# johnnovak/nim-raytracer

Measured on AMD Instinct MI355X. Metric: Mray/s (primary+shadow) on bunny.geom 1080p/256spp; 1/2/4/8-GPU scaling, higher is better.
Workload: dtype f32; 1 GPU; C3: bunny.geom baked x30 + ground plane, mesh-bunny.nim lights/camera, 1920x1080, akGrid 16x16 = 256 spp, fp32, one whole-frame call per step on one GPU; every step builds its camera-dependent data on the device; width=1920, height=1080, spp=256, triangles=69451, bvh_nodes=21204, primary_rays_per_frame=530841600, parallelism=bands1, bvh_builder=host binned SAH

## Files before the change

include/rtmi.h:

```cpp
#ifndef RTMI_H
#define RTMI_H

#include <stddef.h>
#include <stdint.h>

#ifdef __cplusplus
extern "C" {
#endif

#define RTMI_ABI_VERSION 1

enum {
  RT_OK = 0,
  RT_E_INVALID = -1,
  RT_E_UNSUPPORTED = -2,
  RT_E_DEVICE = -3,
  RT_E_NOMEM = -4,
  RT_E_IO = -5
};


enum rt_geom_type { RT_SPHERE = 0, RT_PLANE = 1, RT_BOX = 2, RT_MESH = 3 };

enum rt_light_type { RT_DISTANT_LIGHT = 0, RT_POINT_LIGHT = 1 };
// ... 63 lines not shown
  int32_t max_ray_depth;
  int32_t precision;
  uint64_t seed;
  uint32_t flags;
  uint32_t reserved;
} rt_options;

#define RT_FLAG_ANYHIT_SHADOWS 0x1u
#define RT_FLAG_COUNT_TRAVERSAL 0x2u
#define RT_FLAG_NO_REORDER 0x4u
#define RT_FLAG_NO_BINNING 0x8u
#define RT_FLAG_NO_SPLIT 0x10u
#define RT_FLAG_NO_BATCH 0x20u
#define RT_FLAG_BATCH_FALLBACK 0x40u
#define RT_FLAG_NO_LEAN1 0x80u
#define RT_FLAG_NO_GEN1 0x100u
#define RT_FLAG_NO_STATS 0x200u
#define RT_FLAG_NO_MIX 0x400u
#define RT_FLAG_TIMING 0x800u
#define RT_FLAG_NO_OBJ_BATCH 0x1000u
#define RT_FLAG_COMPACT 0x2000u
#define RT_FLAG_F64_PER_LANE 0x4000u
#define RT_FLAG_NO_UNIFORM 0x8000u

typedef struct rt_stats {
  uint64_t num_primary_rays;
  uint64_t num_intersection_tests;
  uint64_t num_intersection_hits;
  uint64_t num_shadow_rays;
  uint64_t num_reflection_rays;
} rt_stats;

typedef struct rt_traversal_counters {
  uint64_t wave_node_fetches;
  uint64_t wave_tri_fetches;
  uint64_t lane_node_visits;
  uint64_t lane_tri_tests;
} rt_traversal_counters;

typedef struct rt_scene_info {
  int64_t num_objects, num_lights, num_meshes;
  int64_t num_triangles;
  int64_t num_bvh_nodes;
  int32_t max_bvh_depth;
  int32_t device;
  int64_t device_bytes;
// ... 84 lines not shown
int rt_queue_try_recv(rt_queue *q, rt_response *out);
int rt_queue_pending(rt_queue *q);
int rt_queue_reset(rt_queue *q);
int rt_queue_shutdown(rt_queue *q);
int rt_queue_destroy(rt_queue *q);


int rt_ppm_encode_device(const float *d_fb, int32_t width, int32_t height,
                         int32_t bits, int32_t srgb, void *d_out,
                         void *hip_stream);
int64_t rt_ppm_payload_bytes(int32_t width, int32_t height, int32_t bits);
int rt_ppm_header(int32_t width, int32_t height, int32_t bits, char *buf,
                  int32_t buf_len);

int rt_rgba_encode_device(const float *d_fb, int32_t width, int32_t height,
                          uint8_t alpha, void *d_out, void *stream);

int rt_scene_last_counters(rt_scene *scene, rt_traversal_counters *out);

int rt_scene_last_split(rt_scene *scene, int64_t *lean_groups, int64_t *general_groups);
int rt_scene_last_batch(rt_scene *scene, int64_t *batched_groups, int64_t *fallback_groups);
int rt_scene_last_lean_kernel(rt_scene *scene, int32_t *kind);
int rt_scene_last_uniform(rt_scene *scene, int32_t *lit, int32_t *sky);


int rt_mat4_inverse(const double m[16], double out[16]);

int rt_load_geom(const char *path, int64_t *num_triangles, double *vertices);

#define RT_OBJ_SLASH_INDICES 0x1u
int rt_load_obj(const char *path, uint32_t flags, int64_t *num_vertices,
                double *vertices, int64_t *num_faces, int32_t *faces);

int rt_write_geom(const char *path, const double *vertices,
                  int64_t num_vertices, const int32_t *faces,
                  int64_t num_faces);

#ifdef __cplusplus
}
#endif

#endif
```

nim-raytracer_amd/csrc/rt_common.h:

```cpp
#pragma once
#include <stdint.h>
#include <stdlib.h>

namespace rtmi {

inline const char* diag_env(const char* name) {
#ifdef RTMI_DIAG
  return getenv(name);
#else
  (void)name;
  return nullptr;
#endif
}

enum : int32_t { GEOM_SPHERE = 0, GEOM_PLANE = 1, GEOM_BOX = 2, GEOM_MESH = 3 };
enum : int32_t { LIGHT_DISTANT = 0, LIGHT_POINT = 1 };
enum : int32_t { XF_IDENTITY = 0, XF_TRANSLATE = 1, XF_GENERAL = 2 };
enum : int32_t { RT_DEV_FLAG_COUNT = 0x2, RT_DEV_FLAG_FALLBACK = 0x40, RT_DEV_FLAG_NO_OBJ_BATCH = 0x1000 };

constexpr int kMaxBvhDepth = 60;
constexpr int kLeafMax = 4;
constexpr int kMaxShadeLevels = 8;
constexpr int kStatSlots = 10;

// ... 162 lines not shown
  float e2[3];
  float v0;
  float inv_h;
  float rmax;
  int32_t gu, gv;
  int32_t off_base;
  int32_t ent_base;
  int32_t pad[2];
};
static_assert(sizeof(LightGrid) == 64, "LightGrid must be 64 bytes");

struct alignas(16) FLight {
  int32_t type;
  float ci[3];
  float v[3];
  float pad;
};

constexpr uint32_t kPixCount = 0x00FFFFFFu;

constexpr int kLeanClsShift = 29;
constexpr int32_t kLeanIdxMask = (1 << kLeanClsShift) - 1;
enum : int { kUniMixed = 0, kUniLit = 1, kUniSky = 2 };

struct LTri;
struct FastParams {
  const FObj* objs;
  const FObjX* objx;
  const FMesh* meshes;
  const FLight* lights;
  const BvhNode* tree;
  const float* normals;
  const int32_t* pix_slots;
  const uint32_t* pix_cnt;
  const LightGrid* grids;
  const int32_t* grid_off;
  const int32_t* grid_ent;
  const unsigned long long* obj_pix;
  const LightGrid* obj_grids;
  const unsigned long long* obj_grid_mask;
  unsigned long long obj_off_grid;
  const uint32_t* pix_info;
  float* fb;
  unsigned long long* partials;
  unsigned int* queue;
  const int32_t* order;
// ... 96 lines not shown
```

nim-raytracer_amd/csrc/rt_fast.h:

```cpp
#pragma once
#include <hip/hip_runtime.h>

#include "rt_common.h"
#include "rt_sampling.h"

#ifndef RT_CONST
#if defined(__HIP_DEVICE_COMPILE__)
#define RT_CONST __attribute__((address_space(4)))
#else
#define RT_CONST
#endif
#endif



#include "rt_occupancy.h"

namespace rtmi {
namespace fast {

enum : unsigned {
  F_SPHERE = 1u, F_BOX = 2u, F_PLANE = 4u, F_MESH = 8u,
  F_XF_GENERAL = 16u,
  F_POINT = 32u,
// ... 2069 lines not shown
        irr_add(E[k], L.ci, vis ? fmaxf(dot3(N[k], sd), 0.0f) : 0.0f);
      }
    }
  }
  p = params();
  const RT_CONST FObjX& mx = at(p->objx, mesh);
  const RT_CONST FObjX& px_ = at(p->objx, po);
  const F3 am = f3(mx.albedo_pi[0], mx.albedo_pi[1], mx.albedo_pi[2]);
  const F3 ap = f3(px_.albedo_pi[0], px_.albedo_pi[1], px_.albedo_pi[2]);
  const F3 bg = f3(p->bg[0], p->bg[1], p->bg[2]);
#pragma unroll
  for (int k = 0; k < S; ++k) {
    const bool lt = lane_in(litm[k]);
    const F3 alb = f3(hm[k] ? am.x : ap.x, hm[k] ? am.y : ap.y, hm[k] ? am.z : ap.z);
    const F3 a = mul3(alb, E[k]);
    acc_add3(acc, lt ? a.x : bg.x, lt ? a.y : bg.y, lt ? a.z : bg.z);
  }
  wi.v[STAT_PRIMARY] += (unsigned)(64 * S);
  wi.v[STAT_SHADOW] += (unsigned)NL * nlit;
  wi.v[STAT_HITS] += wave_sum(hitl);
  return true;
}

template <unsigned F>
__device__ __forceinline__ LdsF* sample_table(KP p, const GroupPix& gp, float* sample_lds, int wib, int L) {
  LdsF* tb = nullptr;
  if ((F & F_STOCHASTIC) && p->aa_kind >= 3) {
    const int m = p->grid_m, spp = p->spp;
    const uint64_t key = rng_pixel_key(p->seed, gp.x, gp.y);
    tb = (LdsF*)sample_lds + ((size_t)(wib * (64 / L) + (lane_id_fresh() >> p->log2_lanes)) * 2 * spp);
    volatile LdsF* t = tb;
    for (int e = gp.sub; e < spp; e += L) {
      double a, b;
      canonical_entry(key, m, e, a, b);
      t[e] = (float)a;
      t[spp + e] = (float)b;
    }
    const uint64_t bx = 2 * (uint64_t)spp;
    const uint64_t by = bx + (p->aa_kind == 3 ? (uint64_t)spp : (uint64_t)m);
    if (gp.sub < m) {
      const int i = gp.sub;
      for (int j = 0; j < m; ++j) {
        const int k = rng_pick(rng_draw(key, p->aa_kind == 3 ? bx + (uint64_t)j * m + i : bx + (uint64_t)j), j, m);
        const float a = t[j * m + i], b = t[k * m + i];
        t[j * m + i] = b;
        t[k * m + i] = a;
// ... 930 lines not shown
    }
    qj = __builtin_amdgcn_readfirstlane(qj_next);
    if (lane == 0) qj_next = (int)atomicAdd(head, 1u);
    g = qj * p->shards + shard;
  }
  p = params();
  const int lane = (int)__lane_id();
  flush_stats(ws, lds_tot[wib], lane);
  const int wave = (int)(blockIdx.x * (blockDim.x >> 6) + threadIdx.x / 64u);
  if (lane < kStatSlots) p->partials[(size_t)wave * kStatSlots + lane] = lds_tot[wib][lane];
}

#ifndef RTMI_GEN1_WAVES
#define RTMI_GEN1_WAVES 7
#endif
template <int NL>
__device__ __forceinline__ void gen1_loop(KP p, LdsF* ls, Stats32& ws, unsigned long long* tot, int& nflush) {
  constexpr unsigned F = F_PLANE | F_MESH;
  WorkQ<RTMI_GEN_RUN> wq;
  int g = wq.start(p->queue, p->shards, list_items(p->list_n, p->ngroups, 1));
  while (g >= 0) {
    p = params();
    const int iters = p->iters;
    const int gg = cp(p->order)[g];
    GroupPix gp = group_pixel(p, gg, lane_id_fresh());
    gp.valid = true;
    gp.x = __builtin_amdgcn_readfirstlane(gp.x);
    gp.y = __builtin_amdgcn_readfirstlane(gp.y);
    gp.out_row = __builtin_amdgcn_readfirstlane(gp.out_row);
    const int pu = __builtin_amdgcn_readfirstlane(gp.y * p->width + gp.x);
    const unsigned pinfo = at(p->pix_info, pu);
    Acc acc;
    acc.v = f3(0.0f, 0.0f, 0.0f);
    Stats32 wi;
#pragma unroll
    for (int k = 0; k < kStatSlots; ++k) wi.v[k] = 0u;
    bool ok = (pinfo & kPixCount) <= (1u << p->slot_lg);
    for (int it = 0; ok && it < iters; it += kGenBatch) ok = gen1_batch<kGenBatch, NL>(p, gp, pu, it, pinfo, acc, wi);
    if (params()->flags & RT_DEV_FLAG_FALLBACK) ok = false;
    if (ok) {
      ws.v[STAT_PRIMARY] += wi.v[STAT_PRIMARY];
      ws.v[STAT_SHADOW] += wi.v[STAT_SHADOW];
      ws.v[STAT_HITS] += wi.v[STAT_HITS];
#if defined(RTMI_DIAG_GEN_COUNT) || defined(RTMI_DIAG_LANES)
      for (int q = STAT_NODE_FETCH; q <= STAT_LANE_TRIS; ++q) ws.v[q] += wi.v[q];
#endif
    } else {
      acc.v = f3(0.0f, 0.0f, 0.0f);
      ws.v[STAT_GEN_FALLBACK] += 1u;
      for (int i2 = 0; i2 < iters; ++i2) {
        p = params();
        const int s = i2 * 64 + gp.sub;
        const F3 d = camera_dir<F>(p, gp, s, nullptr);
        const F3 o = f3(p->cam[0], p->cam[1], p->cam[2]);
        ws.v[STAT_PRIMARY] += 64u;
        shade_path<false, F, false>(p, o, d, true, gp.y * p->width + gp.x, pinfo, ls, acc, ws);
      }
    }
    p = params();
    finish_item(p, gp, acc.v, 64);
    const int lane = lane_id_fresh();
// ... 58 lines not shown
```

nim-raytracer_amd/csrc/rt_frame.h:

```cpp
#pragma once
#include <stdint.h>

#include "rt_bins_geom.h"
#include "rt_common.h"

namespace rtmi {

constexpr int kFrameMaxPlanes = 8;

struct FrameRows {
  int32_t mode, y0, nrows, step, band_h, rank, world, height;
};
__host__ __device__ inline bool frame_has_row(const FrameRows& r, int y) {
  if (y < 0 || y >= r.height) return false;
  if (r.mode == 0) {
    const int d = y - r.y0;
    return d >= 0 && d < r.nrows * r.step && d % r.step == 0;
  }
  return (y / r.band_h) % r.world == r.rank;
}
__host__ __device__ inline bool frame_meets_rows(const FrameRows& r, int ylo, int yhi) {
  ylo = ylo < 0 ? 0 : ylo;
  yhi = yhi < r.height - 1 ? yhi : r.height - 1;
  if (ylo > yhi) return false;
// ... 38 lines not shown
struct HugeFace {
  int32_t rec, pad;
  int32_t r[4];
  double pr[6];
};

struct RecordsLaunch {
  int32_t mode, y0, nrows, ncols, step, max_step, band_h, rank, world, width, height, ngroups;
  uint32_t* info;
  int32_t nplanes, nl;
  uint32_t have;
  bg::SkipCam cam;
  bg::SkipPlaneC planes[kFrameMaxPlanes];
  const LightGrid* grids;
  const int32_t* sat;
  int64_t sat_off[8];
  int32_t records;
  int32_t split;
  uint32_t full;
  int32_t* lean;
  int32_t* heavy;
  int32_t* ctr;
  bg::UniformCam uni;
  uint32_t* uni_cls;
};

struct FrameLaunch {
  const DevBinTri* tris;
  int32_t nf;
  bg::PixCam cam;
  FrameRows rows;
  int32_t* cnt;
  int32_t* slots;
  int32_t slot_lg;
  HugeFace* huge;
  int32_t parity;
  RecordsLaunch r;
  uint8_t* tile_bits;
  unsigned long long* tile_cls;
  int32_t tiles_x, ntiles;
  unsigned int* zero;
  int32_t nzero;
  int32_t diag;
};

struct DevObjBox {
// ... 24 lines not shown
```

nim-raytracer_amd/csrc/rt_frame.hip:

```cpp
#include <cstdlib>
#include <hip/hip_runtime.h>

#include <algorithm>

#include "rt_bins.h"
#include "rt_frame.h"

namespace rtmi {
namespace {

__device__ __forceinline__ unsigned lane_rank(unsigned long long m) {
  return __builtin_amdgcn_mbcnt_hi((unsigned)(m >> 32), __builtin_amdgcn_mbcnt_lo((unsigned)m, 0u));
}

struct LaunchPix {
  int x, y;
  bool valid, drawn;
};
__device__ __forceinline__ LaunchPix launch_pixel(const RecordsLaunch& a, int j, int k) {
  LaunchPix r;
  r.x = j * a.step;
  r.valid = j < a.ncols && k < a.nrows;
  if (a.mode == 0) {
    r.y = a.y0 + k * a.step;
// ... 257 lines not shown
  for (int off = 32; off >= 1; off >>= 1) {
    const unsigned lo = (unsigned)__shfl_xor((int)(unsigned)v, off);
    const unsigned hi = (unsigned)__shfl_xor((int)(unsigned)(v >> 32), off);
    v += ((unsigned long long)hi << 32) | lo;
  }
  if (lane == 0) wpart[w] = v;
  int cls[kChunkTiles];
#pragma unroll
  for (int i = 0; i < kChunkTiles; ++i) {
    cls[i] = px[i].valid ? pixel_class(r, px[i], inf[i]) : 0;
    const unsigned long long ml = __ballot(cls[i] == 1), mh = __ballot(cls[i] == 2);
    if (lane == 0) wsum[i][w] = ((unsigned long long)__popcll(ml) << 32) | __popcll(mh);
  }
  __syncthreads();
  unsigned long long base = wpart[0] + wpart[1] + wpart[2] + wpart[3];
#pragma unroll
  for (int i = 0; i < kChunkTiles; ++i) {
    const int t = t0 + i;
    const unsigned long long ml = __ballot(cls[i] == 1), mh = __ballot(cls[i] == 2);
    unsigned long long b = base;
    for (int q = 0; q < w; ++q) b += wsum[i][q];
    const int bx = t % a.tiles_x, by = t / a.tiles_x;
    const int g = (by * kTileH + w) * r.ncols + bx * kTileW + lane;
    const int uc = r.uni.on && cls[i] == 1 ? bg::uniform_class(r.uni, px[i].x, px[i].y) : kUniMixed;
    const unsigned long long mul = __ballot(uc == kUniLit), mus = __ballot(uc == kUniSky);
    if (r.uni.on && lane == 0 && t < a.ntiles)
      r.uni_cls[t * kTileH + w] = (uint32_t)__popcll(mul) << 16 | (uint32_t)__popcll(mus);
    if (cls[i] == 1) r.lean[(int)(b >> 32) + (int)lane_rank(ml)] = g | (uc << kLeanClsShift);
    if (cls[i] == 2) r.heavy[(int)(b & 0xffffffffull) + (int)lane_rank(mh)] = g;
    base += wsum[i][0] + wsum[i][1] + wsum[i][2] + wsum[i][3];
  }
  if ((int)blockIdx.x == (int)gridDim.x - 1) {
    const int nl = (int)(base >> 32), nh = (int)(base & 0xffffffffull);
    if (tid == 0) {
      r.ctr[FC_LEAN] = nl;
      r.ctr[FC_HEAVY] = nh;
    }
    const int end = nl == 0 ? 64 : (nl + 63) / 64 * 64;
    for (int e = nl + tid; e < end; e += 256) r.lean[e] = -1;
  }
}

__global__ __launch_bounds__(512) void k_frame_obj_rects(const ObjMaskLaunch a) {
  __shared__ int alw[64];
  const int t = (int)threadIdx.x, i = t >> 3, c = t & 7;
  bool proj = false, bad = false;
  double px = 0.0, py = 0.0;
  if (i < a.nobj) {
    const DevObjBox& b = a.objs[i];
    proj = !b.always;
    const double pw[3] = {(c & 1) ? b.hi[0] : b.lo[0], (c & 2) ? b.hi[1] : b.lo[1], (c & 4) ? b.hi[2] : b.lo[2]};
    double pc[3];
// ... 108 lines not shown
```

nim-raytracer_amd/csrc/rtmi.cpp:

```cpp
#include <hip/hip_runtime.h>

#include <algorithm>
#include <array>
#include <atomic>
#include <chrono>
#include <cmath>
#include <cstdarg>
#include <cstdio>
#include <cstdlib>
#include <cstring>
#include <memory>
#include <mutex>
#include <set>
#include <thread>
#include <string>
#include <vector>

#include "../../include/rtmi.h"
#include "rt_bins.h"
#include "rt_bvh.h"
#include "rt_common.h"
#include "rt_frame.h"

using namespace rtmi;
// ... 210 lines not shown
  bool has_grids = false;
  std::vector<GridOcc> grid_occ;
  std::vector<LightGridHost> grid_host;
  std::vector<SkipPlane> skip_planes;
  bool skippable = false;
  DevBuf<DevBinTri> bin_dev;
  double mesh_lo[3] = {0, 0, 0}, mesh_hi[3] = {0, 0, 0};
  DevBuf<int32_t> sat_dev;
  int64_t sat_off[8] = {};
  struct Frame {
    int w = 0, h = 0;
    DevBuf<int32_t> cnt, slots, lean, heavy, ctr, orect;
    DevBuf<uint32_t> info, uni_cls;
    int uni_rows = 0;
    DevBuf<unsigned long long> omask, status;
    DevBuf<HugeFace> huge;
    DevBuf<unsigned char> tiles;
    int slot_lg = -1;
    int want_lg = slot_lg_env();
    uint32_t calls = 0;
    bool counted = false;
    bool listed = false;
    bool uniform = false;
    hipEvent_t built = nullptr;
    hipEvent_t used = nullptr;
    bool used_rec = false;
    int id = 0;
    void invalidate() { w = h = 0; }
    size_t bytes() const {
      return cnt.bytes() + slots.bytes() + lean.bytes() + heavy.bytes() + ctr.bytes() + orect.bytes() +
             info.bytes() + uni_cls.bytes() + omask.bytes() + status.bytes() + huge.bytes() + tiles.bytes();
    }
    void release() {
      cnt.release(); slots.release(); lean.release(); heavy.release(); ctr.release(); orect.release();
      info.release(); uni_cls.release(); omask.release(); status.release(); huge.release(); tiles.release();
      slot_lg = -1;
      w = h = 0;
    }
  } fr, fr2;
  std::vector<ObjBox> obj_boxes;
  bool objbins = false;
  DevBuf<LightGrid> obj_grids;
  DevBuf<unsigned long long> obj_grid_mask;
  unsigned long long obj_off_grid = 0;
  bool has_obj_grids = false;
  DevBuf<DevObjBox> objbox_dev;
// ... 1070 lines not shown
  u.on = 1;
  u.m = p.grid_m;
  u.cam_a = p.cam_a;
  u.cam_b = p.cam_b;
  u.cam_c = p.cam_c;
  u.cam_d = p.cam_d;
  u.c4 = p.cam[4];
  u.c7 = p.cam[7];
  u.c10 = p.cam[10];
  u.st = p.sample_step;
  u.of = p.sample_off;
  u.nroy = nroy;
  bool ok = p.bias >= 1e-30f &&
            (double)p.bias > 16.0 * 1.1920928955078125e-7 *
                                 ((double)std::fabs(oy) + (double)std::fabs(ty) + (double)std::fabs(nroy));
  for (int l = 0; l < p.nlight; ++l) {
    const float sdy = -s->h_light_vy[(size_t)l];
    ok = ok && sdy > 1e-6f && sdy <= 1e6f;
  }
  u.lit_ok = ok ? 1 : 0;
}

void records_launch(rt_scene* s, const rt_options* o, const Mapping& mp, const FastParams& p, bool records,
                    bool split, bool uniform, RecordsLaunch& r) {
  std::memset(&r, 0, sizeof r);
  r.mode = mp.mode;
  r.y0 = mp.y0;
  r.nrows = mp.nrows;
  r.ncols = mp.ncols;
  r.step = mp.step;
  r.max_step = mp.max_step;
  r.band_h = mp.band_h;
  r.rank = mp.rank;
  r.world = mp.world;
  r.width = o->width;
  r.height = o->height;
  r.ngroups = p.ngroups;
  r.info = s->fr.info.p;
  r.records = records ? 1 : 0;
  if (records && s->skippable && s->skip_planes.size() <= (size_t)kFrameMaxPlanes) {
    std::vector<bg::SkipPlaneC> pcs;
    if (skip_camera(s->skip_planes, s->mesh_w2o, s->c2w, s->fov, o->width, o->height, o->bias, &r.cam, &pcs)) {
      r.nplanes = (int32_t)pcs.size();
      std::copy(pcs.begin(), pcs.end(), r.planes);
      r.nl = std::min(8, s->nlight);
      for (int l = 0; l < r.nl; ++l) r.have |= s->grid_occ[(size_t)l].g.gu > 0 ? 1u << l : 0u;
      r.grids = s->grids.p;
      r.sat = s->sat_dev.p;
      for (int l = 0; l < 8; ++l) r.sat_off[l] = s->sat_off[l];
    }
  }
  r.split = split ? 1 : 0;
  r.full = s->nlight >= 32 ? ~0u : (1u << s->nlight) - 1u;
  r.lean = s->fr.lean.p;
  r.heavy = s->fr.heavy.p;
  r.ctr = s->fr.ctr.p;
  if (split && uniform) {
    uniform_cam(s, p, r.uni);
    r.uni_cls = s->fr.uni_cls.p;
  }
}

int frame_build(rt_scene* s, const rt_options* o, const Mapping& mp, const FastParams& p, bool records, bool split,
                bool uniform, unsigned int* zero, int nzero, hipStream_t st, bool* ok, bool* zeroed) {
  *ok = false;
  *zeroed = false;
  if (!s->binnable || s->bin_tris.empty()) return RT_OK;
  FrameLaunch a;
  std::memset(&a, 0, sizeof a);
  if (!pixel_camera(s->mesh_o2w, s->mesh_w2o, s->c2w, s->fov, o->width, o->height, &a.cam)) return RT_OK;
  for (int c = 0; c < 8; ++c) {
    const double q[3] = {(c & 1) ? s->mesh_hi[0] : s->mesh_lo[0], (c & 2) ? s->mesh_hi[1] : s->mesh_lo[1],
                         (c & 4) ? s->mesh_hi[2] : s->mesh_lo[2]};
    double pw[3], pc[3];
    bg::xform_point(s->mesh_o2w, q, pw);
    bg::xform_point(a.cam.w2c, pw, pc);
    if (!(pc[2] < -1e-9 * (1.0 + std::fabs(pc[0]) + std::fabs(pc[1])))) return RT_OK;
  }
  int rc = frame_buffers(s, o->width, o->height, st);
  if (rc) return rc;
  rt_scene::Frame& f = s->fr;
  a.tris = s->bin_dev.p;
  a.nf = (int32_t)s->bin_tris.size();
  a.rows = frame_rows(mp, o->height);
  a.cnt = f.cnt.p;
  a.slots = f.slots.p;
  a.slot_lg = f.slot_lg;
  a.huge = f.huge.p;
  a.parity = (int32_t)(f.calls++ & 1u);
  records_launch(s, o, mp, p, records, split, uniform, a.r);
  a.tile_bits = f.tiles.p;
  a.tile_cls = f.status.p;
  static const int diag_b2 = rtmi::diag_env("RTMI_DIAG_B2") ? std::atoi(rtmi::diag_env("RTMI_DIAG_B2")) : 0;
  a.diag = diag_b2;
  a.tiles_x = (mp.ncols + 63) / 64;
  a.ntiles = a.tiles_x * ((mp.nrows + 3) / 4);
  a.zero = zero;
  a.nzero = nzero;
  if ((rc = rtmi_frame_build(&a, st))) {
    f.invalidate();
    return fail(RT_E_DEVICE, "frame build launch failed: %s", hipGetErrorString((hipError_t)rc));
  }
  f.listed = true;
  f.uniform = a.r.uni.on != 0;
  f.uni_rows = a.ntiles * 4;
  *zeroed = zero != nullptr;
  *ok = true;
  return RT_OK;
}

int frame_obj_masks(rt_scene* s, const rt_options* o, const Mapping& mp, hipStream_t st, bool* ok) {
  *ok = false;
  ObjMaskLaunch a;
  std::memset(&a, 0, sizeof a);
  static const double kIdentity[16] = {1, 0, 0, 0, 0, 1, 0, 0, 0, 0, 1, 0, 0, 0, 0, 1};
  bg::PixCam pc;
  if (!pixel_camera(kIdentity, kIdentity, s->c2w, s->fov, o->width, o->height, &pc)) return RT_OK;
  int rc = frame_buffers(s, o->width, o->height, st);
  if (rc) return rc;
  a.objs = s->objbox_dev.p;
  a.nobj = s->nobj;
  a.width = o->width;
  a.height = o->height;
  std::memcpy(a.w2c, pc.w2c, sizeof a.w2c);
  a.cam_a = pc.cam_a;
  a.cam_c = pc.cam_c;
  a.margin = kPixelMargin;
// ... 133 lines not shown
  if (!binning || pl.L < 16 || !sampler_in_pixel(o->aa_kind)) return RT_OK;
  int rc;
  bool lists = false, masks = false;
  static const char* cost_dump = rtmi::diag_env("RTMI_COST_DUMP");
  const unsigned sub = f32_subset(s, o);
  const bool want_split = !(o->flags & (RT_FLAG_NO_SPLIT | RT_FLAG_COUNT_TRAVERSAL)) && !p.cost && !cost_dump &&
                          s->nlight <= 8 && rtmi_lean_f32_blocks_per_cu(sub, f32_table_lds(s, o)) > 0;
  const bool records = pl.L == 64;
  *split = records && want_split && !p.order;
  hipStream_t bs = st;
  if (s->pipe) {
    bs = s->bstream;
    if (s->fr.used_rec) HIP_TRY(hipStreamWaitEvent(bs, s->fr.used, 0));
  }
  auto join = [&]() -> int {
    if (bs != st) {
      HIP_TRY(hipEventRecord(s->fr.built, bs));
      HIP_TRY(hipStreamWaitEvent(st, s->fr.built, 0));
    }
    return RT_OK;
  };
  const bool uniform = *split && lean1_ok(s, o, p, sub) && !(o->flags & (RT_FLAG_NO_LEAN1 | RT_FLAG_NO_UNIFORM)) &&
                       rtmi_lean1_quads() && (long long)mp.ncols * mp.nrows <= (long long)kLeanIdxMask;
  if ((rc = frame_build(s, o, mp, p, records, *split, uniform, zero, nzero, bs, &lists, zeroed))) {
    join();
    return rc;
  }
  if (lists) {
    p.pix_slots = s->fr.slots.p;
    p.pix_cnt = s->fr.info.p;
    p.slot_lg = s->fr.slot_lg;
    if (records) p.pix_info = s->fr.info.p;
  } else {
    *split = false;
  }
  if (s->objbins) {
    if ((rc = frame_obj_masks(s, o, mp, bs, &masks))) {
      join();
      return rc;
    }
    if (masks) p.obj_pix = s->fr.omask.p;
  }
  return join();
}

template <class R>
void fill_params(rt_scene* s, const PrecisionData<R>& pd, const rt_options* o, const Mapping& mp, float* fb,
// ... 73 lines not shown

bool mix_policy() {
  static const int force = rtmi::diag_env("RTMI_MIX") ? std::atoi(rtmi::diag_env("RTMI_MIX")) : -1;
  return force != 0;
}

bool lean1_ok(const rt_scene* s, const rt_options* o, const FastParams& p, unsigned sub) {
  return sub == SUB_MESH && p.nobj == 2 && p.shadow_mesh >= 0 &&
         (p.nlight == 1 || p.nlight == 2) && !p.has_point_light && p.aa_kind == RT_AA_GRID &&
         p.log2_grid_m >= 0 && p.log2_grid_m <= 6 && p.lanes_per_px == 64 && p.spp % 256 == 0 &&
         p.iters * 64 == p.spp && p.iters % 4 == 0 && s->nobj == 2;
}

int launch(rt_scene* s, const rt_options* o, const Mapping& mp, float* d_out, hipStream_t st, bool reduce,
           unsigned int* zero, int nzero) {
  int blocks = 1;
  auto clear = [&]() -> int {
    if (nzero > 0) HIP_TRY(hipMemsetAsync(zero, 0, (size_t)nzero * sizeof(unsigned int), st));
    return RT_OK;
  };
  s->fr.counted = false;
  s->fr.listed = false;
  s->fr.uniform = false;
  s->pending_reduce = 0;
  s->last_lean = 0;
  s->last_lean_kind = 0;
  s->last_general = 0;
  s->last_batched = 0;
  if (o->precision == RT_FP64) {
    if (int rc = clear()) return rc;
    RenderParams<double> p;
    fill_params<double>(s, s->f64, o, mp, d_out, p, &blocks);
    s->last_general = p.ngroups;
    if (p.ngroups == 0) return RT_OK;
    if (p.aa_kind >= RT_AA_JITTERED) {
      const size_t need = (size_t)blocks * 256 * 2 * (size_t)p.spp;
      if (s->f64_tables.n < need) {
        HIP_TRY(hipStreamSynchronize(st));
        int rc = s->f64_tables.alloc(need);
        if (rc) return rc;
      }
      p.sample_scratch = s->f64_tables.p;
    }
    s->last_lean = 0;
    s->last_lean_kind = 0;
    s->last_general = p.ngroups;
    s->last_batched = 0;
    const bool binning = !(o->flags & (RT_FLAG_NO_BINNING | RT_FLAG_COUNT_TRAVERSAL));
    bool lists = false;
    if (binning && sampler_in_pixel(o->aa_kind) && s->skippable) {
      FastParams pf;
      std::memset(&pf, 0, sizeof pf);
      bool zeroed = false;
      if (int rc = frame_build(s, o, mp, pf, true, false, false, nullptr, 0, st, &lists, &zeroed)) return rc;
      if (lists) p.pix_info = s->fr.info.p;
    }
    const int px64 = o->aa_kind == RT_AA_GRID && p.spp >= 64 && !(o->flags & (RT_FLAG_F64_PER_LANE | RT_FLAG_COUNT_TRAVERSAL))
                         ? (s->any_reflective && o->max_ray_depth >= 1 ? 2 : 1)
                         : 0;
    if (px64) {
      if (lists) {
        p.pix_slots = s->fr.slots.p;
        p.slot_lg = s->fr.slot_lg;
        p.lean_plane = s->lean64_plane;
      }
      if (binning && s->has_grids) {
        p.grids = s->grids.p;
        p.grid_off = s->grid_off.p;
        p.grid_ent = s->grid_ent.p;
        if (!s->sh64_ready && s->shadow_mesh >= 0) {
          if (int rc = s->sh64.alloc(s->grid_ent.n)) return rc;
          for (int li = 0; li < s->nlight && li < (int)s->grid_host.size(); ++li) {
            const LightGridHost& lg = s->grid_host[(size_t)li];
            if (lg.g.gu <= 0 || lg.ent.empty()) continue;
            const int e = rtmi_build_sh64(s->f64.objects.p, s->shadow_mesh, s->f64.lights.p, li,
                                          s->grid_ent.p + lg.g.ent_base, (int)lg.ent.size(), s->f64.tris.p,
                                          (int32_t)s->num_nodes, s->sh64.p + lg.g.ent_base, st);
// ... 412 lines not shown
  *general = c[FC_HEAVY];
  return RT_OK;
}
}

extern "C" int rt_scene_last_split(rt_scene* s, int64_t* lean_groups, int64_t* general_groups) {
  if (!s || !lean_groups || !general_groups) return fail(RT_E_INVALID, "null argument");
  std::lock_guard<std::mutex> lk(s->mu);
  return last_lists(s, lean_groups, general_groups);
}

extern "C" int rt_scene_last_uniform(rt_scene* s, int32_t* lit, int32_t* sky) {
  if (!s || !lit || !sky) return fail(RT_E_INVALID, "null argument");
  std::lock_guard<std::mutex> lk(s->mu);
  *lit = 0;
  *sky = 0;
  if (!s->fr.counted || !s->fr.uniform) return RT_OK;
  DeviceGuard g(s->device);
  std::vector<uint32_t> c((size_t)s->fr.uni_rows);
  HIP_TRY(hipEventSynchronize(s->done));
  HIP_TRY(hipMemcpy(c.data(), s->fr.uni_cls.p, c.size() * sizeof(uint32_t), hipMemcpyDeviceToHost));
  for (const uint32_t v : c) {
    *lit += (int32_t)(v >> 16);
    *sky += (int32_t)(v & 0xffffu);
  }
  return RT_OK;
}

extern "C" int rt_scene_last_lean_kernel(rt_scene* s, int32_t* kind) {
  if (!s || !kind) return fail(RT_E_INVALID, "null argument");
  std::lock_guard<std::mutex> lk(s->mu);
  *kind = s->last_lean_kind;
  return RT_OK;
}

extern "C" int rt_scene_last_batch(rt_scene* s, int64_t* batched_groups, int64_t* fallback_groups) {
  if (!s || !batched_groups || !fallback_groups) return fail(RT_E_INVALID, "null argument");
  std::lock_guard<std::mutex> lk(s->mu);
  *batched_groups = s->last_batched;
  if (s->last_batched < 0) {
    int64_t lean = 0;
    const int rc = last_lists(s, &lean, batched_groups);
    if (rc) return rc;
  }
  *fallback_groups = s->last_fallback;
  return RT_OK;
}

// ... 96 lines not shown
```

nim-raytracer_amd/rtmi/abi.py:

```python
import ctypes as C

RTMI_ABI_VERSION = 1

RT_OK = 0
RT_E_INVALID = -1
RT_E_UNSUPPORTED = -2
RT_E_DEVICE = -3
RT_E_NOMEM = -4
RT_E_IO = -5

RT_SPHERE, RT_PLANE, RT_BOX, RT_MESH = 0, 1, 2, 3
RT_DISTANT_LIGHT, RT_POINT_LIGHT = 0, 1
RT_AA_NONE, RT_AA_GRID, RT_AA_JITTERED, RT_AA_MULTI_JITTERED, RT_AA_CORRELATED_MULTI_JITTERED = range(5)
RT_FP32, RT_FP64 = 0, 1
RT_FLAG_ANYHIT_SHADOWS = 0x1
RT_FLAG_COUNT_TRAVERSAL = 0x2
RT_FLAG_NO_REORDER = 0x4
RT_FLAG_NO_BINNING = 0x8
RT_FLAG_NO_SPLIT = 0x10
RT_FLAG_NO_BATCH = 0x20
RT_FLAG_BATCH_FALLBACK = 0x40
RT_FLAG_NO_LEAN1 = 0x80
RT_FLAG_NO_GEN1 = 0x100
RT_FLAG_NO_STATS = 0x200
RT_FLAG_NO_MIX = 0x400
RT_FLAG_TIMING = 0x800
RT_FLAG_NO_OBJ_BATCH = 0x1000
RT_FLAG_COMPACT = 0x2000
RT_FLAG_F64_PER_LANE = 0x4000
RT_FLAG_NO_UNIFORM = 0x8000
RT_BVH_SAH = 0
RT_OBJ_SLASH_INDICES = 0x1
RT_BVH_PLOC = 1

_d16 = C.c_double * 16
_d3 = C.c_double * 3


class rt_mesh_desc(C.Structure):
    _fields_ = [
        ("vertices", C.POINTER(C.c_double)),
        ("num_vertices", C.c_int64),
        ("faces", C.POINTER(C.c_int32)),
        ("num_faces", C.c_int64),
        ("normals", C.POINTER(C.c_double)),
    ]


class rt_object_desc(C.Structure):
    _fields_ = [
        ("type", C.c_int32),
        ("mesh", C.c_int32),
        ("object_to_world", _d16),
# ... 106 lines not shown
    "rt_version": (C.c_int, []),
    "rt_build_source_hash": (C.c_char_p, []),
    "rt_last_error": (C.c_char_p, []),
    "rt_init": (C.c_int, [C.c_int]),
    "rt_device_count": (C.c_int, []),
    "rt_scene_create": (C.c_int, [C.POINTER(rt_scene_desc), C.POINTER(_P)]),
    "rt_scene_destroy": (C.c_int, [_P]),
    "rt_scene_get_info": (C.c_int, [_P, C.POINTER(rt_scene_info)]),
    "rt_scene_set_camera": (C.c_int, [_P, C.POINTER(C.c_double), C.c_double]),
    "rt_render_lines": (C.c_int, [_P, C.POINTER(rt_options), C.POINTER(C.c_float), C.c_int32,
                                  C.c_int32, C.c_int32, C.c_int32, C.c_int32, C.c_int32,
                                  C.POINTER(rt_stats)]),
    "rt_render_lines_device": (C.c_int, [_P, C.POINTER(rt_options), _P, C.c_int32, C.c_int32,
                                         C.c_int32, C.c_int32, _P, C.POINTER(rt_stats)]),
    "rt_render_bands_device": (C.c_int, [_P, C.POINTER(rt_options), _P, C.c_int32, C.c_int32,
                                         C.c_int32, _P, C.POINTER(rt_stats)]),
    "rt_unshard_bands_device": (C.c_int, [_P, _P, C.c_int32, C.c_int32, C.c_int32, C.c_int32, _P]),
    "rt_band_rows": (C.c_int, [C.c_int32, C.c_int32, C.c_int32, C.POINTER(C.c_int32)]),
    "rt_scene_last_counters": (C.c_int, [_P, C.POINTER(rt_traversal_counters)]),
    "rt_scene_last_split": (C.c_int, [_P, C.POINTER(C.c_int64), C.POINTER(C.c_int64)]),
    "rt_scene_last_lean_kernel": (C.c_int, [_P, C.POINTER(C.c_int32)]),
    "rt_scene_last_batch": (C.c_int, [_P, C.POINTER(C.c_int64), C.POINTER(C.c_int64)]),
    "rt_scene_last_uniform": (C.c_int, [_P, C.POINTER(C.c_int32), C.POINTER(C.c_int32)]),
    "rt_mat4_inverse": (C.c_int, [C.POINTER(C.c_double), C.POINTER(C.c_double)]),
    "rt_load_geom": (C.c_int, [C.c_char_p, C.POINTER(C.c_int64), C.POINTER(C.c_double)]),
    "rt_ppm_encode_device": (C.c_int, [_P, C.c_int32, C.c_int32, C.c_int32, C.c_int32, _P, _P]),
    "rt_ppm_payload_bytes": (C.c_int64, [C.c_int32, C.c_int32, C.c_int32]),
    "rt_rgba_encode_device": (C.c_int, [_P, C.c_int32, C.c_int32, C.c_uint8, _P, _P]),
    "rt_ppm_header": (C.c_int, [C.c_int32, C.c_int32, C.c_int32, C.c_char_p, C.c_int32]),
    "rt_load_obj": (C.c_int, [C.c_char_p, C.c_uint32, C.POINTER(C.c_int64), C.POINTER(C.c_double),
                              C.POINTER(C.c_int64), C.POINTER(C.c_int32)]),
    "rt_write_geom": (C.c_int, [C.c_char_p, C.POINTER(C.c_double), C.c_int64, C.POINTER(C.c_int32), C.c_int64]),
    "rt_scene_last_stats": (C.c_int, [_P, C.POINTER(rt_stats)]),
    "rt_scene_last_timing": (C.c_int, [_P, C.POINTER(C.c_double), C.POINTER(C.c_double)]),
    "rt_multi_create": (C.c_int, [C.POINTER(rt_scene_desc), C.POINTER(C.c_int32), C.c_int32, C.c_int32,
                                  C.POINTER(_P)]),
    "rt_render_frame_multi_device": (C.c_int, [_P, C.POINTER(rt_options), _P, C.POINTER(rt_stats)]),
    "rt_render_frame_multi": (C.c_int, [_P, C.POINTER(rt_options), C.POINTER(C.c_float), C.c_int32, C.c_int32,
                                        C.POINTER(rt_stats)]),
    "rt_multi_set_camera": (C.c_int, [_P, C.POINTER(C.c_double), C.c_double]),
    "rt_multi_destroy": (C.c_int, [_P]),
    "rt_queue_create": (C.c_int, [_P, C.POINTER(_P)]),
    "rt_queue_start": (C.c_int, [_P]),
    "rt_queue_stop": (C.c_int, [_P]),
    "rt_queue_state": (C.c_int, [_P]),
    "rt_queue_is_ready": (C.c_int, [_P]),
# ... 20 lines not shown
```

nim-raytracer_amd/rtmi/renderer.py:

```python
import contextlib
import ctypes as C
import threading

import numpy as np

from . import abi, glm
from ._lib import RtmiError, check, lib
from .scene import Options, Scene, Stats, flatten


def initRenderer(device=0):
    check(lib().rt_init(int(device)))


def device_count():
    return int(lib().rt_device_count())


class DeviceScene:

    def __init__(self, scene: Scene, device=0, bvh_builder=abi.RT_BVH_SAH):
        initRenderer(device)
        self.device = device
        self.scene = scene
# ... 56 lines not shown
        check(lib().rt_render_bands_device(self.h, C.byref(o), C.c_void_p(ptr), int(band_h), int(rank),
                                           int(world), _stream(stream), C.byref(st) if stats else None))
        return Stats.from_c(st) if stats else None

    def last_pipelined(self):
        f = lib().rtmi_test_last_pipelined
        f.restype = C.c_int
        f.argtypes = [C.c_void_p, C.POINTER(C.c_int32)]
        s = C.c_int32()
        r = f(self.h, C.byref(s))
        if r < 0:
            raise RuntimeError("rtmi_test_last_pipelined failed")
        return bool(r)

    def last_split(self):
        a, b = C.c_int64(), C.c_int64()
        check(lib().rt_scene_last_split(self.h, C.byref(a), C.byref(b)))
        return int(a.value), int(b.value)

    def last_uniform(self):
        a, b = C.c_int32(), C.c_int32()
        check(lib().rt_scene_last_uniform(self.h, C.byref(a), C.byref(b)))
        return int(a.value), int(b.value)

    def last_lean_kernel(self):
        k = C.c_int32()
        check(lib().rt_scene_last_lean_kernel(self.h, C.byref(k)))
        return int(k.value) & 15

    def last_compacted(self):
        k = C.c_int32()
        check(lib().rt_scene_last_lean_kernel(self.h, C.byref(k)))
        return bool(int(k.value) & 16)

    def last_lean_lanes(self):
        k = C.c_int32()
        check(lib().rt_scene_last_lean_kernel(self.h, C.byref(k)))
        return int(k.value) >> 8

    def last_batch(self):
        a, b = C.c_int64(), C.c_int64()
        check(lib().rt_scene_last_batch(self.h, C.byref(a), C.byref(b)))
        return int(a.value), int(b.value)

    def last_timing(self):
        a, b = C.c_double(), C.c_double()
# ... 353 lines not shown
```

Before: 2.316 million Mray/s.

## Add ground-plane fast path for general pixel groups that only see the floor

During frame list building, heavy (general) pixel groups whose footprint is classified as uniformly lit ground are tagged with a ground bit. The general kernel then sends these groups to a specialized ground1_batch routine. It computes the plane hit analytically and traces only shadow rays through the light grid, skipping full primary BVH traversal and the generic shading path. The trade-offs are extra per-group classification work, a new code path with fallbacks when the grid is unsafe, and repacked uniform-class counters (the sky count now uses 8 bits).

```diff
diff --git a/include/rtmi.h b/include/rtmi.h
--- a/include/rtmi.h
+++ b/include/rtmi.h
@@ -109,6 +109,7 @@
 #define RT_FLAG_COMPACT 0x2000u
 #define RT_FLAG_F64_PER_LANE 0x4000u
 #define RT_FLAG_NO_UNIFORM 0x8000u
+#define RT_FLAG_NO_GROUND1 0x10000u
 
 typedef struct rt_stats {
   uint64_t num_primary_rays;
@@ -239,6 +240,7 @@
 int rt_scene_last_batch(rt_scene *scene, int64_t *batched_groups, int64_t *fallback_groups);
 int rt_scene_last_lean_kernel(rt_scene *scene, int32_t *kind);
 int rt_scene_last_uniform(rt_scene *scene, int32_t *lit, int32_t *sky);
+int rt_scene_last_ground(rt_scene *scene, int32_t *ground);
 
 
 int rt_mat4_inverse(const double m[16], double out[16]);
diff --git a/nim-raytracer_amd/csrc/rt_common.h b/nim-raytracer_amd/csrc/rt_common.h
--- a/nim-raytracer_amd/csrc/rt_common.h
+++ b/nim-raytracer_amd/csrc/rt_common.h
@@ -208,6 +208,7 @@
 constexpr int kLeanClsShift = 29;
 constexpr int32_t kLeanIdxMask = (1 << kLeanClsShift) - 1;
 enum : int { kUniMixed = 0, kUniLit = 1, kUniSky = 2 };
+constexpr int32_t kGenGroundBit = 1 << kLeanClsShift;
 
 struct LTri;
 struct FastParams {
diff --git a/nim-raytracer_amd/csrc/rt_fast.h b/nim-raytracer_amd/csrc/rt_fast.h
--- a/nim-raytracer_amd/csrc/rt_fast.h
+++ b/nim-raytracer_amd/csrc/rt_fast.h
@@ -2115,6 +2115,138 @@
   return true;
 }
 
+#ifndef RTMI_GROUND_BATCH
+#define RTMI_GROUND_BATCH 4
+#endif
+constexpr int kGroundBatch = RTMI_GROUND_BATCH;
+static_assert(kGroundBatch == 1 || kGroundBatch == 2 || kGroundBatch == 4, "iters is a multiple of 4");
+template <int S, int NL>
+__device__ __forceinline__ bool ground1_batch(KP p, const GroupPix& gp, int it0, unsigned pinfo, Acc& acc,
+                                              Stats32& wi) {
+  p = params();
+  const int mesh = p->shadow_mesh, po = 1 - mesh;
+  const FObj mob = at(p->objs, mesh);
+  F3 ro[S];
+  {
+    const F3 o = f3(p->cam[0], p->cam[1], p->cam[2]);
+    const float nroy = -(o.y + at(p->objs, po).t[1]), bias = p->bias;
+    const int mm = p->grid_m - 1, lg = p->log2_grid_m;
+    const float st = p->sample_step, of = p->sample_off;
+    const float px = (float)gp.x + __builtin_fmaf((float)(gp.sub & mm), st, of);
+    const float cx = (px - p->cam_b) * p->cam_a;
+    const float q0 = __builtin_fmaf(cx, cx, 1.0f);
+    const float ax = __builtin_fmaf(cx, p->cam[3], -p->cam[9]), ay = __builtin_fmaf(cx, p->cam[4], -p->cam[10]),
+                az = __builtin_fmaf(cx, p->cam[5], -p->cam[11]);
+#pragma unroll
+    for (int k = 0; k < S; ++k) {
+      const int s = (it0 + k) * 64 + gp.sub;
+      const float py = (float)gp.y + __builtin_fmaf((float)(s >> lg), st, of);
+      const float cy = (p->cam_d - py) * p->cam_c;
+      const float rl = rsq(__builtin_fmaf(cy, cy, q0));
+      const F3 d = f3(__builtin_fmaf(cy, p->cam[6], ax) * rl, __builtin_fmaf(cy, p->cam[7], ay) * rl,
+                      __builtin_fmaf(cy, p->cam[8], az) * rl);
+      const float th = nroy * rcp(d.y);
+      const F3 hw = f3(__builtin_fmaf(d.x, th, o.x), __builtin_fmaf(d.y, th, o.y), __builtin_fmaf(d.z, th, o.z));
+      const F3 so = f3(__builtin_fmaf(0.0f, bias, hw.x), __builtin_fmaf(1.0f, bias, hw.y),
+                       __builtin_fmaf(0.0f, bias, hw.z));
+      ro[k] = f3(so.x + mob.t[0], so.y + mob.t[1], so.z + mob.t[2]);
+    }
+  }
+  unsigned long long occ[NL][S];
+  unsigned nocc = 0u;
+  const unsigned skipw = pinfo >> 24;
+#pragma unroll
+  for (int li = 0; li < NL; ++li) {
+#pragma unroll
+    for (int k = 0; k < S; ++k) occ[li][k] = 0ull;
+    if (((skipw >> li) & 1u) != 0u || mob.root < 0) continue;
+    p = params();
+    const FLight L = at(p->lights, li);
+    const F3 sd = f3(-L.v[0], -L.v[1], -L.v[2]);
+    unsigned long long pm[S], anyp = 0ull;
+#pragma unroll
+    for (int k = 0; k < S; ++k) {
+      pm[k] = bal(mesh_gate(mob, slab_ray(ro[k], sd)));
+      anyp |= pm[k];
+    }
+    if (anyp == 0ull) continue;
+    const KP q = params();
+    if (!q->grids || q->grids[li].gu <= 0) return false;
+    const RT_CONST LightGrid& G = cp(q->grids)[li];
+    F3 rd[S];
+    float stop[S], tc[S], best[S];
+    unsigned long long unused[S];
+    int cell[S];
+    unsigned long long todo[S], left = 0ull, unsafe = 0ull;
+#pragma unroll
+    for (int k = 0; k < S; ++k) {
+      const bool part = lane_in(pm[k]);
+      rd[k] = sd;
+      stop[k] = __uint_as_float(__float_as_uint(finf()) - 1u);
+      tc[k] = part ? finf() : -1.0f;
+      best[k] = part ? finf() : 0.0f;
+      unused[k] = 0ull;
+      const F3 r = ro[k];
+      const float gu = __builtin_fmaf(r.x, G.e1[0], __builtin_fmaf(r.y, G.e1[1], r.z * G.e1[2]));
+      const float gv = __builtin_fmaf(r.x, G.e2[0], __builtin_fmaf(r.y, G.e2[1], r.z * G.e2[2]));
+      const float fu = (gu - G.u0) * G.inv_h, fv = (gv - G.v0) * G.inv_h;
+      const bool safe = fmaxf(fmaxf(fabsf(r.x), fabsf(r.y)), fabsf(r.z)) <= G.rmax;
+      const bool on = fu >= 0.0f && fu < (float)G.gu && fv >= 0.0f && fv < (float)G.gv;
+      cell[k] = safe && on ? G.off_base + (int)fv * G.gu + (int)fu : -1;
+      todo[k] = bal(part && cell[k] >= 0);
+      unsafe |= bal(part && !safe);
+      left |= todo[k];
+    }
+    if (unsafe != 0ull) return false;
+    const int32_t* bent = q->grid_ent + G.ent_base;
+    while (left != 0ull) {
+      int kb = -1;
+#pragma unroll
+      for (int k = S - 1; k >= 0; --k)
+        if (todo[k]) kb = __builtin_amdgcn_readlane(cell[k], (int)__builtin_ctzll(todo[k]));
+      unsigned fl = 0u;
+      unsigned long long own[S];
+      left = 0ull;
+#pragma unroll
+      for (int k = 0; k < S; ++k) {
+        own[k] = bal(cell[k] == kb) & todo[k];
+        todo[k] &= ~own[k];
+        left |= todo[k];
+        fl |= own[k] != 0ull ? (1u << k) : 0u;
+      }
+      (void)list_search_batch<S, false>(q, bent, cp(q->grid_off)[kb], cp(q->grid_off)[kb + 1], fl, ro, rd, stop, own,
+                                        unused, best, tc, nullptr, grid_rec_of(q, li, G));
+    }
+#pragma unroll
+    for (int k = 0; k < S; ++k) {
+      occ[li][k] = pm[k] & bal(__float_as_uint(best[k]) != __float_as_uint(finf()));
+      nocc += pc(occ[li][k]);
+    }
+  }
+  p = params();
+  F3 E[S];
+#pragma unroll
+  for (int k = 0; k < S; ++k) E[k] = f3(0.0f, 0.0f, 0.0f);
+#pragma unroll
+  for (int li = 0; li < NL; ++li) {
+    const FLight L = at(p->lights, li);
+    const float ndl = fmaxf(dot3(f3(0.0f, 1.0f, 0.0f), f3(-L.v[0], -L.v[1], -L.v[2])), 0.0f);
+#pragma unroll
+    for (int k = 0; k < S; ++k) irr_add(E[k], L.ci, lane_in(occ[li][k]) ? 0.0f : ndl);
+  }
+  const RT_CONST FObjX& px_ = at(p->objx, po);
+  const F3 ap = f3(px_.albedo_pi[0], px_.albedo_pi[1], px_.albedo_pi[2]);
+#pragma unroll
+  for (int k = 0; k < S; ++k) {
+    const F3 a = mul3(ap, E[k]);
+    acc_add3(acc, a.x, a.y, a.z);
+  }
+  wi.v[STAT_PRIMARY] += (unsigned)(64 * S);
+  wi.v[STAT_SHADOW] += (unsigned)(NL * 64 * S);
+  wi.v[STAT_HITS] += (unsigned)(64 * S) + nocc;
+  return true;
+}
+
 template <unsigned F>
 __device__ __forceinline__ LdsF* sample_table(KP p, const GroupPix& gp, float* sample_lds, int wib, int L) {
   LdsF* tb = nullptr;
@@ -3091,7 +3223,15 @@
   while (g >= 0) {
     p = params();
     const int iters = p->iters;
-    const int gg = cp(p->order)[g];
+    const int ge = cp(p->order)[g];
+    const bool gnd = (ge & kGenGroundBit) != 0 && p->ngroups <= kLeanIdxMask;
+    const int gg = gnd ? ge & kLeanIdxMask : ge;
+#ifdef RTMI_DIAG_NOGROUND
+    if (gnd) {
+      g = wq.next();
+      continue;
+    }
+#endif
     GroupPix gp = group_pixel(p, gg, lane_id_fresh());
     gp.valid = true;
     gp.x = __builtin_amdgcn_readfirstlane(gp.x);
@@ -3105,7 +3245,11 @@
 #pragma unroll
     for (int k = 0; k < kStatSlots; ++k) wi.v[k] = 0u;
     bool ok = (pinfo & kPixCount) <= (1u << p->slot_lg);
-    for (int it = 0; ok && it < iters; it += kGenBatch) ok = gen1_batch<kGenBatch, NL>(p, gp, pu, it, pinfo, acc, wi);
+    if (gnd) {
+      for (int it = 0; ok && it < iters; it += kGroundBatch) ok = ground1_batch<kGroundBatch, NL>(p, gp, it, pinfo, acc, wi);
+    } else {
+      for (int it = 0; ok && it < iters; it += kGenBatch) ok = gen1_batch<kGenBatch, NL>(p, gp, pu, it, pinfo, acc, wi);
+    }
     if (params()->flags & RT_DEV_FLAG_FALLBACK) ok = false;
     if (ok) {
       ws.v[STAT_PRIMARY] += wi.v[STAT_PRIMARY];
diff --git a/nim-raytracer_amd/csrc/rt_frame.h b/nim-raytracer_amd/csrc/rt_frame.h
--- a/nim-raytracer_amd/csrc/rt_frame.h
+++ b/nim-raytracer_amd/csrc/rt_frame.h
@@ -84,6 +84,7 @@
   int32_t* heavy;
   int32_t* ctr;
   bg::UniformCam uni;
+  int32_t ground;
   uint32_t* uni_cls;
 };
 
diff --git a/nim-raytracer_amd/csrc/rt_frame.hip b/nim-raytracer_amd/csrc/rt_frame.hip
--- a/nim-raytracer_amd/csrc/rt_frame.hip
+++ b/nim-raytracer_amd/csrc/rt_frame.hip
@@ -303,12 +303,15 @@
     for (int q = 0; q < w; ++q) b += wsum[i][q];
     const int bx = t % a.tiles_x, by = t / a.tiles_x;
     const int g = (by * kTileH + w) * r.ncols + bx * kTileW + lane;
-    const int uc = r.uni.on && cls[i] == 1 ? bg::uniform_class(r.uni, px[i].x, px[i].y) : kUniMixed;
-    const unsigned long long mul = __ballot(uc == kUniLit), mus = __ballot(uc == kUniSky);
-    if (r.uni.on && lane == 0 && t < a.ntiles)
-      r.uni_cls[t * kTileH + w] = (uint32_t)__popcll(mul) << 16 | (uint32_t)__popcll(mus);
+    const bool lean_c = r.uni.on && cls[i] == 1, gen_c = r.ground && cls[i] == 2 && (inf[i] & kPixCount) == 0u;
+    const int uc = lean_c || gen_c ? bg::uniform_class(r.uni, px[i].x, px[i].y) : kUniMixed;
+    const bool gnd = gen_c && uc == kUniLit;
+    const unsigned long long mul = __ballot(lean_c && uc == kUniLit), mus = __ballot(lean_c && uc == kUniSky);
+    const unsigned long long mug = __ballot(gnd);
+    if ((r.uni.on || r.ground) && lane == 0 && t < a.ntiles)
+      r.uni_cls[t * kTileH + w] = (uint32_t)__popcll(mul) << 16 | (uint32_t)__popcll(mug) << 8 | (uint32_t)__popcll(mus);
     if (cls[i] == 1) r.lean[(int)(b >> 32) + (int)lane_rank(ml)] = g | (uc << kLeanClsShift);
-    if (cls[i] == 2) r.heavy[(int)(b & 0xffffffffull) + (int)lane_rank(mh)] = g;
+    if (cls[i] == 2) r.heavy[(int)(b & 0xffffffffull) + (int)lane_rank(mh)] = gnd ? g | kGenGroundBit : g;
     base += wsum[i][0] + wsum[i][1] + wsum[i][2] + wsum[i][3];
   }
   if ((int)blockIdx.x == (int)gridDim.x - 1) {
diff --git a/nim-raytracer_amd/csrc/rtmi.cpp b/nim-raytracer_amd/csrc/rtmi.cpp
--- a/nim-raytracer_amd/csrc/rtmi.cpp
+++ b/nim-raytracer_amd/csrc/rtmi.cpp
@@ -256,6 +256,7 @@
     bool counted = false;
     bool listed = false;
     bool uniform = false;
+    bool ground = false;
     hipEvent_t built = nullptr;
     hipEvent_t used = nullptr;
     bool used_rec = false;
@@ -1372,7 +1373,7 @@
 }
 
 void records_launch(rt_scene* s, const rt_options* o, const Mapping& mp, const FastParams& p, bool records,
-                    bool split, bool uniform, RecordsLaunch& r) {
+                    bool split, bool uniform, bool ground, RecordsLaunch& r) {
   std::memset(&r, 0, sizeof r);
   r.mode = mp.mode;
   r.y0 = mp.y0;
@@ -1405,14 +1406,16 @@
   r.lean = s->fr.lean.p;
   r.heavy = s->fr.heavy.p;
   r.ctr = s->fr.ctr.p;
-  if (split && uniform) {
+  if (split && (uniform || ground)) {
     uniform_cam(s, p, r.uni);
+    r.uni.on = uniform ? 1 : 0;
+    r.ground = ground ? 1 : 0;
     r.uni_cls = s->fr.uni_cls.p;
   }
 }
 
 int frame_build(rt_scene* s, const rt_options* o, const Mapping& mp, const FastParams& p, bool records, bool split,
-                bool uniform, unsigned int* zero, int nzero, hipStream_t st, bool* ok, bool* zeroed) {
+                bool uniform, bool ground, unsigned int* zero, int nzero, hipStream_t st, bool* ok, bool* zeroed) {
   *ok = false;
   *zeroed = false;
   if (!s->binnable || s->bin_tris.empty()) return RT_OK;
@@ -1438,7 +1441,7 @@
   a.slot_lg = f.slot_lg;
   a.huge = f.huge.p;
   a.parity = (int32_t)(f.calls++ & 1u);
-  records_launch(s, o, mp, p, records, split, uniform, a.r);
+  records_launch(s, o, mp, p, records, split, uniform, ground, a.r);
   a.tile_bits = f.tiles.p;
   a.tile_cls = f.status.p;
   static const int diag_b2 = rtmi::diag_env("RTMI_DIAG_B2") ? std::atoi(rtmi::diag_env("RTMI_DIAG_B2")) : 0;
@@ -1453,6 +1456,7 @@
   }
   f.listed = true;
   f.uniform = a.r.uni.on != 0;
+  f.ground = a.r.ground != 0;
   f.uni_rows = a.ntiles * 4;
   *zeroed = zero != nullptr;
   *ok = true;
@@ -1632,7 +1636,11 @@
   };
   const bool uniform = *split && lean1_ok(s, o, p, sub) && !(o->flags & (RT_FLAG_NO_LEAN1 | RT_FLAG_NO_UNIFORM)) &&
                        rtmi_lean1_quads() && (long long)mp.ncols * mp.nrows <= (long long)kLeanIdxMask;
-  if ((rc = frame_build(s, o, mp, p, records, *split, uniform, zero, nzero, bs, &lists, zeroed))) {
+  const bool ground = *split && lean1_ok(s, o, p, sub) &&
+                      !(o->flags & (RT_FLAG_NO_BATCH | RT_FLAG_NO_GEN1 | RT_FLAG_NO_GROUND1)) && p.grids &&
+                      rtmi_gen_f32_blocks_per_cu(sub, f32_table_lds(s, o)) > 0 &&
+                      (long long)mp.ncols * mp.nrows <= (long long)kLeanIdxMask;
+  if ((rc = frame_build(s, o, mp, p, records, *split, uniform, ground, zero, nzero, bs, &lists, zeroed))) {
     join();
     return rc;
   }
@@ -1752,6 +1760,7 @@
   s->fr.counted = false;
   s->fr.listed = false;
   s->fr.uniform = false;
+  s->fr.ground = false;
   s->pending_reduce = 0;
   s->last_lean = 0;
   s->last_lean_kind = 0;
@@ -1782,7 +1791,7 @@
       FastParams pf;
       std::memset(&pf, 0, sizeof pf);
       bool zeroed = false;
-      if (int rc = frame_build(s, o, mp, pf, true, false, false, nullptr, 0, st, &lists, &zeroed)) return rc;
+      if (int rc = frame_build(s, o, mp, pf, true, false, false, false, nullptr, 0, st, &lists, &zeroed)) return rc;
       if (lists) p.pix_info = s->fr.info.p;
     }
     const int px64 = o->aa_kind == RT_AA_GRID && p.spp >= 64 && !(o->flags & (RT_FLAG_F64_PER_LANE | RT_FLAG_COUNT_TRAVERSAL))
@@ -2241,8 +2250,21 @@
   HIP_TRY(hipMemcpy(c.data(), s->fr.uni_cls.p, c.size() * sizeof(uint32_t), hipMemcpyDeviceToHost));
   for (const uint32_t v : c) {
     *lit += (int32_t)(v >> 16);
-    *sky += (int32_t)(v & 0xffffu);
-  }
+    *sky += (int32_t)(v & 0xffu);
+  }
+  return RT_OK;
+}
+
+extern "C" int rt_scene_last_ground(rt_scene* s, int32_t* ground) {
+  if (!s || !ground) return fail(RT_E_INVALID, "null argument");
+  std::lock_guard<std::mutex> lk(s->mu);
+  *ground = 0;
+  if (!s->fr.counted || !s->fr.ground) return RT_OK;
+  DeviceGuard g(s->device);
+  std::vector<uint32_t> c((size_t)s->fr.uni_rows);
+  HIP_TRY(hipEventSynchronize(s->done));
+  HIP_TRY(hipMemcpy(c.data(), s->fr.uni_cls.p, c.size() * sizeof(uint32_t), hipMemcpyDeviceToHost));
+  for (const uint32_t v : c) *ground += (int32_t)((v >> 8) & 0xffu);
   return RT_OK;
 }
 
diff --git a/nim-raytracer_amd/rtmi/abi.py b/nim-raytracer_amd/rtmi/abi.py
--- a/nim-raytracer_amd/rtmi/abi.py
+++ b/nim-raytracer_amd/rtmi/abi.py
@@ -29,6 +29,7 @@
 RT_FLAG_COMPACT = 0x2000
 RT_FLAG_F64_PER_LANE = 0x4000
 RT_FLAG_NO_UNIFORM = 0x8000
+RT_FLAG_NO_GROUND1 = 0x10000
 RT_BVH_SAH = 0
 RT_OBJ_SLASH_INDICES = 0x1
 RT_BVH_PLOC = 1
@@ -181,6 +182,7 @@
     "rt_scene_last_lean_kernel": (C.c_int, [_P, C.POINTER(C.c_int32)]),
     "rt_scene_last_batch": (C.c_int, [_P, C.POINTER(C.c_int64), C.POINTER(C.c_int64)]),
     "rt_scene_last_uniform": (C.c_int, [_P, C.POINTER(C.c_int32), C.POINTER(C.c_int32)]),
+    "rt_scene_last_ground": (C.c_int, [_P, C.POINTER(C.c_int32)]),
     "rt_mat4_inverse": (C.c_int, [C.POINTER(C.c_double), C.POINTER(C.c_double)]),
     "rt_load_geom": (C.c_int, [C.c_char_p, C.POINTER(C.c_int64), C.POINTER(C.c_double)]),
     "rt_ppm_encode_device": (C.c_int, [_P, C.c_int32, C.c_int32, C.c_int32, C.c_int32, _P, _P]),
diff --git a/nim-raytracer_amd/rtmi/renderer.py b/nim-raytracer_amd/rtmi/renderer.py
--- a/nim-raytracer_amd/rtmi/renderer.py
+++ b/nim-raytracer_amd/rtmi/renderer.py
@@ -102,6 +102,11 @@
         a, b = C.c_int32(), C.c_int32()
         check(lib().rt_scene_last_uniform(self.h, C.byref(a), C.byref(b)))
         return int(a.value), int(b.value)
+
+    def last_ground(self):
+        a = C.c_int32()
+        check(lib().rt_scene_last_ground(self.h, C.byref(a)))
+        return int(a.value)
 
     def last_lean_kernel(self):
         k = C.c_int32()
```

After: 2.468 million Mray/s, median of 6. 6.5% higher.
